# huakunyang/SummerTTS

Measured on AMD Instinct MI355X. Metric: audio samples/sec (acoustic model + vocoder, phoneme ids -> int16 PCM on host), single_speaker_fast-shaped synthetic blob, higher is better.
Workload: dtype f32 (decoder trunk convs AND the reverse flow's WaveNet convs (wn_flow.hip, one-utterance calls): fp32 operands as 2 fp16 terms = 22-23 of their 24 mantissa bits, 3 fp16 MFMA products per fp32 product, f32 accumulation -- measured error in `parity`, same tolerance as the exact-fp32 leg; batches addi

## Files before the change

### include/summertts_hip.h

```cpp
#ifndef SUMMERTTS_HIP_H_
#define SUMMERTTS_HIP_H_

#include <stdint.h>

#ifdef __cplusplus
extern "C" {
#endif

typedef struct sts_engine sts_engine;

enum {
    STS_OK = 0,
    STS_EINVAL = -1,
    STS_EMODEL = -2,
    STS_EDEVICE = -3,
    STS_ESTATE = -4
};

int sts_create(const float* blob, int64_t blob_bytes, int device, sts_engine** out);
void sts_destroy(sts_engine* e);

int sts_speaker_num(const sts_engine* e);

typedef struct sts_model_info {
// ... 126 lines not shown
#define STS_EQ_LOWPASS 5
typedef struct sts_eq_band { int32_t type; float freq_hz; float gain_db; float q; } sts_eq_band;
int sts_set_eq(sts_engine* e, int32_t n_bands, const sts_eq_band* bands);
int sts_get_eq(const sts_engine* e, int32_t* n_bands, sts_eq_band* bands, int32_t capacity);
int sts_eq_check(int32_t rate, int32_t n_bands, const sts_eq_band* bands);
int sts_eq_design(int32_t rate, int32_t n_bands, const sts_eq_band* bands, double* coeffs);
int sts_eq_apply(int device, const float* x, const int64_t* lengths, int32_t B, int32_t rate, int32_t n_bands,
                 const sts_eq_band* bands, float* y, int16_t* pcm);
int sts_set_eq_streaming(sts_engine* e, int enable);
int sts_get_eq_streaming(const sts_engine* e);
int sts_eq_apply_chunked(int device, const float* x, const int64_t* lengths, int32_t B, int32_t rate, int32_t n_bands,
                         const sts_eq_band* bands, const int64_t* bounds, int32_t n_steps, int32_t back, float* y, int16_t* pcm,
                         float* win_y, int64_t win_capacity, int64_t* win_off);
int sts_set_record_taps(sts_engine* e, int enable);
int sts_get_tap(sts_engine* e, const char* name, float** data, int32_t* channels, int64_t* length);
int sts_get_durations(sts_engine* e, int32_t* dur, int64_t capacity);
int sts_set_conv_mode(sts_engine* e, int mode);
int sts_set_conv_math(sts_engine* e, int mode);

enum { STS_DBG_ATTN_BLOCK_MIN_WGS = 1,
       STS_DBG_TAIL_FUSED = 14 ,
       STS_DBG_UPS_ROWPH = 15 ,
       STS_DBG_CHAIN_STREAMS = 13 ,
       STS_DBG_H2P = 11 ,
       STS_DBG_H2P_TILE = 12 ,
       STS_DBG_MEMO_CLEAR = 10 ,
       STS_DBG_PCM_DIRECT = 9 ,
       STS_DBG_DDS_TAIL = 8 ,
       STS_DBG_ATTN_REG = 7 ,
       STS_DBG_LAUNCH_AHEAD = 6 ,
       STS_DBG_FLOW_FUSED = 5  };
enum { STS_DBG_STREAM_RETRY_STEP = 16, STS_DBG_STREAM_DIRECT = 17 };
enum { STS_DBG_POISON = 18 };
int sts_debug_set(sts_engine* e, int key, int value);

typedef struct sts_profile {
    float ms_text_encoder, ms_duration, ms_flow, ms_decoder, ms_total_device;
    float ms_decoder_mfma;
    int32_t decoder_mfma_launches;
    double flops_text_encoder, flops_duration, flops_flow, flops_decoder;
    double flops_decoder_mfma;
    double bytes_decoder_min;
    int64_t frames, samples, phonemes;
    double flops_decoder_mfma_executed;
    double bytes_text_encoder, bytes_duration, bytes_flow;
    float ms_sync_wait_host;
    double flops_decoder_bf16_issued;
    int64_t conv_math_fallbacks;
    int32_t conv_math_pinned;
    int32_t launch_ahead;
    int64_t launch_ahead_misses;
    float us_host_setup;
    float us_host_enqueue;
    float us_host_tail;
    int64_t poison_bytes;
} sts_profile;
int sts_set_profiling(sts_engine* e, int enable);
#define STS_ABI_VERSION 16
int sts_abi_version(void);
int sts_build_flags(void);
int sts_get_profile(const sts_engine* e, sts_profile* p);
int sts_get_profile_ex(const sts_engine* e, void* p, int64_t size_bytes);

int sts_debug_conv1d(int device, const float* x, int32_t Cin, int32_t L, const float* w, const float* bias,
                     int32_t Cout, int32_t k, int32_t pad, int32_t dil, int32_t stride_transposed,
                     int32_t depthwise, float in_slope, int32_t in_act, int mode, float** y, int32_t* Lout);
// ... 97 lines not shown
```

### summertts_amd/csrc/capi.hip

```cpp
#include <stdlib.h>
#include <string.h>

#include <algorithm>
#include <new>
#include <string>
#include <utility>
#include <vector>

#include "engine.hpp"
#include "eq_stream.hpp"
#include "join_stream.hpp"
#include "loud_stream.hpp"

using namespace sts;

struct sts_engine { Engine eng; };

static thread_local std::string g_err;
static int set_err(int code, const std::string& s) { g_err = s; return code; }
#define STS_CAPI_NOT_WHILE_OPEN(e) \
    do { if ((e)->eng.stream_is_open()) return set_err(STS_ESTATE, "a stream is open on this engine (sts_stream_close first)"); } while (0)

extern "C" {

// ... 708 lines not shown
    if (noise_scale_w) *noise_scale_w = e->eng.noise.nsw;
    if (seed) *seed = e->eng.noise.seed;
    return STS_OK;
}
int sts_set_record_taps(sts_engine* e, int enable) { if (!e) return set_err(STS_EINVAL, "null engine"); STS_CAPI_NOT_WHILE_OPEN(e); e->eng.record_taps = enable != 0; return STS_OK; }
int sts_set_conv_math(sts_engine* e, int mode) {
    if (!e) return set_err(STS_EINVAL, "null engine");
    if (mode < 0 || mode > 3) return set_err(STS_EINVAL, "conv math: 0 = split-bf16 (default), 1 = exact fp32, 2 = split-bf16 wherever eligible, 3 = two-term fp16");
    STS_CAPI_NOT_WHILE_OPEN(e);
    e->eng.conv_math = mode;
    e->eng.h2_consecutive = 0; e->eng.h2_disabled = false;
    return STS_OK;
}
int sts_set_conv_mode(sts_engine* e, int mode) { if (!e) return set_err(STS_EINVAL, "null engine"); STS_CAPI_NOT_WHILE_OPEN(e); e->eng.conv_mode = mode; return STS_OK; }
int sts_debug_set(sts_engine* e, int key, int value) {
    if (!e) return set_err(STS_EINVAL, "null engine");
    if (key != STS_DBG_STREAM_RETRY_STEP && key != STS_DBG_POISON) STS_CAPI_NOT_WHILE_OPEN(e);
    switch (key) {
        case STS_DBG_ATTN_BLOCK_MIN_WGS: if (value < 1) return set_err(STS_EINVAL, "threshold must be >= 1"); e->eng.attn_block_min_wgs = value; return STS_OK;
        case STS_DBG_FLOW_FUSED: e->eng.flow_fused = value == 2 || value == 3 ? value : value != 0; return STS_OK;
        case STS_DBG_LAUNCH_AHEAD: if (value < 0 || value > 2) return set_err(STS_EINVAL, "launch_ahead must be 0, 1 or 2"); if ((value == 2) != (e->eng.launch_ahead == 2)) { e->eng.seen_tf_.clear(); e->eng.seen_order_.clear(); } e->eng.launch_ahead = value; return STS_OK;
        case STS_DBG_H2P: e->eng.h2p = value < 0 ? 0 : (value > 4 ? 4 : value); return STS_OK;
        case STS_DBG_H2P_TILE: e->eng.h2p_tile = value; return STS_OK;
        case STS_DBG_CHAIN_STREAMS: e->eng.chain_streams_dbg = value; return STS_OK;
        case STS_DBG_TAIL_FUSED: e->eng.tail_fused = value != 0; return STS_OK;
        case STS_DBG_UPS_ROWPH: e->eng.ups_rowph = value != 0; return STS_OK;
        case STS_DBG_MEMO_CLEAR: e->eng.seen_tf_.clear(); e->eng.seen_order_.clear(); return STS_OK;
        case STS_DBG_ATTN_REG: e->eng.attn_reg = value != 0; return STS_OK;
        case STS_DBG_DDS_TAIL: e->eng.dds_tail = value != 0; return STS_OK;
        case STS_DBG_PCM_DIRECT: e->eng.pcm_direct = value != 0; return STS_OK;
        case STS_DBG_STREAM_RETRY_STEP: e->eng.stream_retry_step = value < 0 ? -1 : value; return STS_OK;
        case STS_DBG_STREAM_DIRECT: e->eng.stream_direct = value != 0; return STS_OK;
        case STS_DBG_POISON: e->eng.poison = (unsigned)value; return STS_OK;
        default: return set_err(STS_EINVAL, "unknown debug key");
    }
}
int sts_set_host_pcm(sts_engine* e, int enable) { if (!e) return set_err(STS_EINVAL, "null engine"); e->eng.host_pcm = enable != 0; return STS_OK; }
int sts_set_profiling(sts_engine* e, int enable) { if (!e) return set_err(STS_EINVAL, "null engine"); e->eng.profiling = enable == 2 ? 2 : (enable != 0 ? 1 : 0); return STS_OK; }

int sts_abi_version(void) { return STS_ABI_VERSION; }

int sts_set_output_rate(sts_engine* e, int32_t rate) {
    if (!e) return set_err(STS_EINVAL, "null engine");
    const int rc = e->eng.set_output_rate(rate);
    return rc == STS_OK ? STS_OK : set_err(rc, e->eng.error());
}
int sts_get_output_rate(const sts_engine* e) {
    if (!e) return set_err(STS_EINVAL, "null engine");
    return e->eng.out_rate;
}
int sts_resample_table(int32_t in_rate, int32_t out_rate, int32_t* P, int32_t* Q, int32_t* taps, float* table, int64_t capacity_floats) {
    ResampleDesign d;
    if (!resample_design(in_rate, out_rate, &d)) return set_err(STS_EINVAL, "rates must be integers in [8000, 48000] with P = out / gcd(in, out) <= 1024");
    const int64_t need = (int64_t)d.P * 2 * d.K;
    if (table && capacity_floats < need) return set_err(STS_EINVAL, "table capacity below P * taps floats");
    if (P) *P = d.P;
    if (Q) *Q = d.Q;
    if (taps) *taps = 2 * d.K;
    if (table) resample_table(d, in_rate, out_rate, table);
    return STS_OK;
}
int sts_set_loudness(sts_engine* e, int mode, float target_lufs, float peak_dbfs) {
    if (!e) return set_err(STS_EINVAL, "null engine");
    const int rc = e->eng.set_loudness(mode, target_lufs, peak_dbfs);
    return rc == STS_OK ? STS_OK : set_err(rc, e->eng.error());
}
// ... 817 lines not shown
```

### summertts_amd/csrc/col_layer.hip

```cpp
#include "kernels.hpp"
#include "devmath.hpp"

#ifndef STS_EXP
#define STS_EXP 0
#endif

namespace sts {

typedef float f32x4 __attribute__((ext_vector_type(4)));

__device__ __forceinline__ int cl_seg_start(const SegView& s, int b) { return (s.off ? s.off[b] : s.ioff) * s.scale + b * s.extra; }
__device__ __forceinline__ int cl_seg_len(const SegView& s, int b) { return (s.off ? s.len[b] : s.ilen) * s.scale + s.extra; }

template <int NSUB, bool TAIL = false>
__global__ __launch_bounds__(64 * NSUB) void col_layer_kernel(ColLayerArgs a) {
    constexpr int C = 16 * NSUB, KQ = C / 4, CG = 4 * NSUB;
    constexpr int KH = KQ > 48 ? KQ / 2 : KQ;
    __shared__ float ys[C * 16];
    __shared__ float red[2][NSUB][16];
    const int b = blockIdx.y;
    const int len = cl_seg_len(a.seg, b);
    const int n0 = blockIdx.x * 16;
    if (n0 >= len) return;
    const size_t base = (size_t)cl_seg_start(a.seg, b);
// ... 128 lines not shown
    for (int r = 0; r < 4; r++) {
        float o = ((v[r] - mean) / den) * e_g[r] + e_b[r];
        if (a.post_gelu && !(STS_EXP & 1)) o = gelu_ref(o);
        if (a.res) o = e_res[r] + o;
        o4[r] = o;
        if (!TAIL) a.y[(size_t)(row0 + r) * a.y_ld + base + pos] = o;
    }
    if constexpr (TAIL) {
    __shared__ float tp[32 * 16], wb[32];
    __shared__ __attribute__((aligned(16))) float wl[C * 32];
#pragma unroll
    for (int r = 0; r < 4; r++) ys[(row0 + r) * 16 + col] = live ? o4[r] : 0.f;
    reinterpret_cast<f32x4*>(wl)[tid] = tw0; reinterpret_cast<f32x4*>(wl)[tid + 64 * NSUB] = tw1;
    if (tid < 32) wb[tid] = t_bias;
    __syncthreads();
    for (int j = tid >> 4; j < 32; j += 4 * NSUB) {
        float acc = 0.f;
#pragma unroll 8
        for (int c = 0; c < C; c++) acc += wl[c * 32 + j] * ys[c * 16 + col];
        acc += wb[j];
        tp[j * 16 + col] = j < 29 ? rq_spline_param(j, acc, a.tp_fs) : 0.f;
    }
    __syncthreads();
    if (tid < 16 && live) {
        float t[29];
#pragma unroll
        for (int j = 0; j < 29; j++) t[j] = tp[j * 16 + tid];
        a.tp_o0[base + pos] = rq_spline_inverse_t(t_in, t);
        a.tp_o1[base + pos] = t_keep;
    }
    }
}

template <int NSUB>
__global__ __launch_bounds__(64 * NSUB) void col_proj_kernel(ColProjArgs a) {
    constexpr int C = 16 * NSUB, KQ = C / 4, CG = 4 * NSUB;
    __shared__ float ys[C * 16];
    __shared__ float red[2][NSUB][16];
    const int b = blockIdx.y;
    const int len = cl_seg_len(a.seg, b);
    const int n0 = blockIdx.x * 16;
    if (n0 >= len) return;
    const size_t base = (size_t)cl_seg_start(a.seg, b);
    const int tid = threadIdx.x, lane = tid & 63, wave = tid >> 6;
    const int col = lane & 15, quad = lane >> 4;
    const int pos = n0 + col;
    const bool live = pos < len;
    const int cg = tid >> 4;

    float v[4], g[4], be[4];
    if (a.ids) {
        int id = live ? a.ids[base + pos] : 0;
        if (id < 0 || id >= a.vocab) id = 0;
#pragma unroll
        for (int i = 0; i < 4; i++) v[i] = live ? a.emb[(size_t)(cg + i * CG) * a.vocab + id] * a.emb_scale : 0.f;
    } else {
#pragma unroll
        for (int i = 0; i < 4; i++) {
            const int c = cg + i * CG;
            g[i] = a.gamma[c]; be[i] = a.beta[c];
            float x0 = live ? a.a[(size_t)c * a.a_ld + base + pos] : 0.f;
            float pb[8];
#pragma unroll
            for (int q = 0; q < 8; q++) pb[q] = (live && q < a.nb) ? a.bp[(size_t)q * a.b_stride + (size_t)c * a.b_ld + base + pos] : 0.f;
            float bs = pb[0];
#pragma unroll
            for (int q = 1; q < 8; q++) bs += pb[q];
            v[i] = x0 + bs;
        }
    }
    f32x4 afa[KQ / 4], afb[KQ / 4];
    auto load_strip = [&](int pass, f32x4 (&dst)[KQ / 4]) {
        const f32x4* wp = reinterpret_cast<const f32x4*>(a.wc) + ((size_t)pass * NSUB + wave) * (KQ / 4) * 64 + lane;
#pragma unroll
        for (int i = 0; i < KQ / 4; i++) dst[i] = wp[(size_t)i * 64];
    };
    load_strip(0, afa);

    if (!a.ids) {
        float s = 0.f, sq = 0.f;
#pragma unroll
        for (int i = 0; i < 4; i++) { s += v[i]; sq += v[i] * v[i]; }
        s += __shfl_xor(s, 16, 64); sq += __shfl_xor(sq, 16, 64);
        s += __shfl_xor(s, 32, 64); sq += __shfl_xor(sq, 32, 64);
        if (quad == 0) { red[0][wave][col] = s; red[1][wave][col] = sq; }
        __syncthreads();
        s = 0.f; sq = 0.f;
#pragma unroll
        for (int k = 0; k < NSUB; k++) { s += red[0][k][col]; sq += red[1][k][col]; }
        const float mean = s / (float)C;
        const float var = sq * (float)(1. / (float)C) - mean * mean;
        const float den = (float)sqrt((double)var + 1e-05);
#pragma unroll
        for (int i = 0; i < 4; i++) v[i] = ((v[i] - mean) / den) * g[i] + be[i];
    }
#pragma unroll
    for (int i = 0; i < 4; i++) {
        const int c = cg + i * CG;
        ys[c * 16 + col] = live ? v[i] : 0.f;
        if (live) a.x_out[(size_t)c * a.x_ld + base + pos] = v[i];
    }
    __syncthreads();

    float bq[KQ];
#pragma unroll
    for (int i = 0; i < KQ; i++) bq[i] = ys[(4 * i + quad) * 16 + col];
    const int rloc = wave * 16 + quad * 4;
    auto run_pass = [&](int pass, const f32x4 (&af)[KQ / 4]) {
        f32x4 acc0 = {0.f, 0.f, 0.f, 0.f}, acc1 = {0.f, 0.f, 0.f, 0.f};
#pragma unroll
        for (int i = 0; i < KQ; i += 2) {
            acc0 = __builtin_amdgcn_mfma_f32_16x16x4f32(af[i / 4][i % 4], bq[i], acc0, 0, 0, 0);
            acc1 = __builtin_amdgcn_mfma_f32_16x16x4f32(af[(i + 1) / 4][(i + 1) % 4], bq[i + 1], acc1, 0, 0, 0);
        }
        if (live) {
#pragma unroll
            for (int r = 0; r < 4; r++) {
                const int row = pass * C + rloc + r;
                if (row < a.Cout) a.y[(size_t)row * a.y_ld + base + pos] = (acc0[r] + acc1[r]) + (a.bias ? a.bias[row] : 0.f);
            }
        }
    };
    for (int pass = 0; pass < a.npass; pass += 2) {
        if (pass + 1 < a.npass) load_strip(pass + 1, afb);
        run_pass(pass, afa);
        if (pass + 1 < a.npass) {
            if (pass + 2 < a.npass) load_strip(pass + 2, afa);
            run_pass(pass + 1, afb);
        }
    }
}

bool col_proj_eligible(const ColProjArgs& a) {
    if (a.C != 32 && a.C != 64 && a.C != 192) return false;
    if (!a.wc || !a.y || !a.x_out || a.npass < 1 || a.npass > 4 || a.Cout > a.npass * a.C || a.Cout <= (a.npass - 1) * a.C) return false;
    if (a.ids) { if (!a.emb || a.vocab <= 0) return false; }
    else if (!a.a || !a.gamma || !a.beta || a.nb < 0 || a.nb > 8 || (a.nb > 0 && !a.bp)) return false;
    return a.max_len > 0 && a.B > 0;
}

void col_proj(const ColProjArgs& a, hipStream_t st) {
    const dim3 grid((a.max_len + 15) / 16, a.B);
    switch (a.C) {
        case 32: hipLaunchKernelGGL((col_proj_kernel<2>), grid, dim3(128), 0, st, a); break;
        case 64: hipLaunchKernelGGL((col_proj_kernel<4>), grid, dim3(256), 0, st, a); break;
        default: hipLaunchKernelGGL((col_proj_kernel<12>), grid, dim3(768), 0, st, a); break;
    }
}

void col_layer_pack(const float* w, int C, float* dst) { col_proj_pack(w, C, C, dst); }
void col_proj_pack(const float* w, int C, int Cout, float* dst) {
    const int nsub = C / 16, kq4 = C / 16, npass = (Cout + C - 1) / C;
    for (int pass = 0; pass < npass; pass++)
        for (int wave = 0; wave < nsub; wave++)
            for (int i4 = 0; i4 < kq4; i4++)
                for (int lane = 0; lane < 64; lane++)
                    for (int e = 0; e < 4; e++) {
                        const int co = pass * C + 16 * wave + (lane & 15), ci = 4 * (4 * i4 + e) + (lane >> 4);
                        dst[((((size_t)pass * nsub + wave) * kq4 + i4) * 64 + lane) * 4 + e] = co < Cout ? w[(size_t)co * C + ci] : 0.f;
                    }
}
bool col_layer_width_ok(int C) { return C == 32 || C == 64 || C == 192 || C == 256; }

bool col_layer_eligible(const ColLayerArgs& a) {
    if (!col_layer_width_ok(a.C)) return false;
    if (!a.wc || !a.g2 || !a.b2 || !a.x || !a.y) return false;
    if (a.dw_w && (!a.g1 || !a.b1 || a.dw_k < 1 || a.dw_k > 3)) return false;
    if (a.xs_w && (!a.dw_w || a.res != a.x)) return false;
    if (a.tp_w && (a.C == 256 || !a.tp_b || !a.tp_o0 || !a.tp_o1 || a.tp_o0 == a.tp_r0 || a.tp_o0 == a.tp_r1 || a.tp_o1 == a.tp_r1)) return false;
    if (a.y == a.x) return false;
    return a.max_len > 0 && a.B > 0;
}

void col_layer(const ColLayerArgs& a, hipStream_t st) {
// ... 19 lines not shown
```

### summertts_amd/csrc/engine.hip

```cpp
#include "run_ctx.hpp"
#include <time.h>
#include "knobs.hpp"
#include "../../include/tts_logger.h"

#include <algorithm>
#include <chrono>
#include <math.h>
#include <new>
#include <stdlib.h>
#include <string.h>
#include <thread>

namespace sts {

#define STS_NOT_WHILE_OPEN(what) \
    do { if (live_) return fail(STS_ESTATE, "a stream is open on this engine (sts_stream_close first): it refuses " what); } while (0)

Engine::~Engine() {
    if (live_) (void)stream_close();
    if (stream) (void)hipStreamSynchronize(stream);
    free_model(model);
    if (arenaT_.base) (void)hipFree(arenaT_.base);
    if (arenaF_.base) (void)hipFree(arenaF_.base);
    if (pinned_) (void)hipHostFree(pinned_);
// ... 561 lines not shown
    for (int b = 0; b < B; b++) { p_ns[b] = c.nz[b].ns; p_nsw[b] = c.nz[b].nsw; p_seed[b] = c.nz[b].seed; }
    int* p_ids = (int*)(p_seed + B);
    for (int b = 0; b < B; b++) memcpy(p_ids + offT[b], ids[b], sizeof(int) * n[b]);
    if (mix) memcpy(p_ids + Ttot, mix_words.data(), sizeof(int) * mix_ints);
    if (gain) memcpy(p_ids + Ttot + mix_ints, gain_words.data(), sizeof(int) * gain_ints);
    if (join) memcpy(p_ids + Ttot + mix_ints + gain_ints, join_sil.data(), sizeof(int) * join_ints);
    int* p_forced = p_ids + Ttot + mix_ints + gain_ints + join_ints;
    if (have_forced) memcpy(p_forced, forced_dur.data(), sizeof(int) * Ttot);
    if (plan) {
        memcpy(p_ids + Ttot + mix_ints + gain_ints + join_ints, plan_rate.data(), sizeof(float) * Ttot);
        memcpy(p_ids + 2 * Ttot + mix_ints + gain_ints + join_ints, plan_fixed.data(), sizeof(int) * Ttot);
        memcpy(p_ids + 3 * Ttot + mix_ints + gain_ints + join_ints, plan_target.data(), sizeof(int) * B);
    }
    HIPCK(hipMemcpyAsync(bt.meta_i, pm, (meta_ints + 5 * (size_t)B + (size_t)Ttot * (have_forced ? 2 : 1) + mix_ints + gain_ints + join_ints + plan_ints) * 4, hipMemcpyHostToDevice, stream));
    if (B > 1) HIPCK(hipEventRecord(ev_setup_, stream));

    static const bool no_inline_seg_knob = exp_flag("STS_NO_INLINE_SEG");
    const bool no_inline_seg = c.no_inline_seg = no_inline_seg_knob;
    const bool inl = c.inl = B == 1 && !no_inline_seg;
    c.ms = M.is_ms == 1;
    lvT.seg = inl ? SegView{nullptr, nullptr, 1, 0, 0, lenT[0]} : SegView{d_offT, d_lenT, 1, 0, 0, 0};
    Lvl& lvB = c.lvB; lvB = Lvl(); lvB.seg = no_inline_seg ? SegView{d_one, d_one + 1, 1, 0, 0, 0} : SegView{nullptr, nullptr, 1, 0, 0, B};
    lvB.nb = 1; lvB.max_len = B; lvB.total = B; lvB.ld = B;

    return STS_OK;
}

int Engine::run_text_encoder(RunCtx& c) {
    RUN_ALIASES(c)
    stage_begin(0);
    static const bool no_colp = exp_flag("STS_NO_COL_LAYER") || exp_flag("STS_NO_COL_PROJ");
    const long colp_blocks = (long)((Ttot + 15) / 16);
    const bool colp_grid = (long)((maxT + 15) / 16) * B <= 512;
    auto produce_x_and_conv = [&](int l, const DConv& c, float* y) {
        ColProjArgs pj;
        memset(&pj, 0, sizeof(pj));
        pj.x_out = bt.x; pj.x_ld = Ttot; pj.wc = c.wc; pj.bias = c.bias_rows; pj.Cout = c.Cout; pj.npass = (c.Cout + H - 1) / H;
        pj.y = y; pj.y_ld = Ttot; pj.C = H; pj.seg = lvT.seg; pj.B = B; pj.max_len = maxT;
        if (l == 0) { pj.ids = bt.ids; pj.emb = M.emb; pj.vocab = M.vocab; pj.emb_scale = sqrtf((float)M.hidden); }
        else { pj.a = bt.x1; pj.a_ld = Ttot; pj.bp = bt.y; pj.b_ld = Ttot; pj.nb = ffn2_slices; pj.b_stride = (long)H * Ttot;
               pj.gamma = M.ln2[l - 1].g; pj.beta = M.ln2[l - 1].b; }
        const bool ok = !no_colp && conv_mode != 1 && colp_grid && (pj.npass == 1 || colp_blocks >= 24) && c.k == 1 && c.Cin == H && M.emb_size == H && c.wc &&
                        (l == 0 || M.ln2[l - 1].C == H) && col_proj_eligible(pj);
        if (ok) {
            flops_[0] += 2.0 * c.macs_per_out * (double)Ttot;
            bytes_[0] += 4.0 * ((double)H * Ttot * (l == 0 ? 1.0 : 2.0 + ffn2_slices) + (double)c.Cout * Ttot + (double)H * c.Cout);
            col_proj(pj, stream);
            return;
        }
        if (l == 0) embed(bt.ids, M.emb, M.vocab, M.emb_size, sqrtf((float)M.hidden), bt.x, Ttot, (int)Ttot, stream);
        else ln(M.ln2[l - 1], bt.x1, bt.y, nullptr, bt.x, lvT, 0, 0, ffn2_slices, (long)H * Ttot);
        conv(c, bt.x, lvT, y, lvT, ConvOpt());
    };
    for (int l = 0; l < M.n_layers; l++) {
        const DMha& a = M.mha[l];
        produce_x_and_conv(l, a.qkv, bt.qkv);
        AttnArgs at;
        memset(&at, 0, sizeof(at));
        at.q = bt.qkv; at.k = bt.qkv + (size_t)H * Ttot; at.v = bt.qkv + (size_t)2 * H * Ttot; at.o = bt.att; at.ld = Ttot;
        at.relk = a.relk; at.relv = a.relv; at.kc = a.kc; at.px = a.px; at.win = a.win; at.nheads = 2;
        at.seg = lvT.seg; at.B = B; at.max_len = maxT; at.block_min_wgs = attn_block_min_wgs; at.attn_reg = attn_reg;
        attention(at, stream);
        flops_[0] += 2.0 * 2.0 * (double)a.ch * (double)maxT * (double)Ttot;
        bytes_[0] += 4.0 * 4.0 * (double)H * (double)Ttot;
        {
            static const bool no_col = exp_flag("STS_NO_COL_LAYER");
            ColLayerArgs g;
            memset(&g, 0, sizeof(g));
            g.x = bt.att; g.x_ld = Ttot; g.wc = a.o.wc; g.bias = a.o.bias;
            g.add = bt.x; g.add_ld = Ttot; g.g2 = M.ln1[l].g; g.b2 = M.ln1[l].b; g.y = bt.x1; g.y_ld = Ttot; g.C = H;
            g.seg = lvT.seg; g.B = B; g.max_len = maxT;
            if (!no_col && conv_mode != 1 && a.o.Cin == H && a.o.Cout == H && a.o.Cin_pad == H && M.ln1[l].C == H && col_layer_eligible(g)) {
                flops_[0] += 2.0 * a.o.macs_per_out * (double)Ttot;
                bytes_[0] += 4.0 * ((double)H * Ttot * 3.0 + (double)H * H);
                col_layer(g, stream);
            } else {
                conv(a.o, bt.att, lvT, bt.y, lvT, ConvOpt());
                ln(M.ln1[l], bt.x, bt.y, nullptr, bt.x1, lvT, 0, 0);
            }
// ... 1 lines not shown
        const DFfn& f = M.ffn[l];
        ConvOpt o1; o1.pad_l = f.ksize == 1 ? 0 : (f.ksize - 1) / 2;
        conv(f.c1, bt.x1, lvT, bt.ffh, lvT, o1);
        ConvOpt o2 = o1; o2.in_act = 1; o2.slope = 0.f;
        o2.kslices = ffn2_slices; o2.kslice_stride = (long)H * Ttot;
        conv(f.c2, bt.ffh, lvT, bt.y, lvT, o2);
    }
    produce_x_and_conv(M.n_layers, M.proj, bt.m);
    if (bt.logs) conv(M.proj_logs, bt.x, lvT, bt.logs, lvT, ConvOpt());
    tap("x_enc", bt.x, H, Ttot, Ttot);
    tap("m", bt.m, C, Ttot, Ttot);
    if (bt.logs) tap("logs", bt.logs, C, Ttot, Ttot);
    mark(1);
    return STS_OK;
}

int Engine::run_durations(RunCtx& c) {
    Model& M = model;
    const int B = c.B; const StreamSpec* const ss = c.ss; const long Ttot = c.Ttot;
    [[maybe_unused]] const int H = c.H, fdp = c.fdp;
    Lvl &lvT = c.lvT, &lvB = c.lvB; BufT& bt = c.bt;
    const size_t up_bytes = c.up_bytes; int* const pm = c.pm; int* const p_offF = c.p_offF; int* const p_lenF = c.p_lenF;
    int* const d_sid = c.d_sid; int* const d_offF = c.d_offF;
    const bool inl = c.inl, ms = c.ms; const int maxT = c.maxT; (void)maxT;

    stage_begin(1);
    if (ms && c.mix) speaker_blend(M.emb_g, M.spk_num, M.gin, d_sid, B, speaker_mix_tab(bt.mix, B, mix_K), bt.g, stream);
    else if (ms) gather_speaker(M.emb_g, M.spk_num, M.gin, d_sid, B, bt.g, stream);

    const float* r_final = nullptr;
    if (M.dur_type == 0) {
        ConvOpt op;
        if (ms) { conv(M.sdp_cond, bt.g, lvB, bt.cond_dp, lvB, ConvOpt()); op.ubias = bt.cond_dp; }
        conv(M.sdp_pre, bt.x, lvT, bt.dh, lvT, op);
        const float* dh = dds(M.sdp_dds, bt.dh, bt.dt1, bt.dt2, lvT);
        conv(M.sdp_proj, dh, lvT, bt.dc, lvT, ConvOpt());
        const float *r0 = nullptr, *r1 = nullptr;
        float *n0 = bt.dr[2], *n1 = bt.dr[3], *s0 = bt.dr[0], *s1 = bt.dr[1];
        if (c.any_nsw) { sdp_noise(lvT.seg, B, maxT, bt.nsw, bt.seed, bt.dr[0], bt.dr[1], stream); r0 = bt.dr[0]; r1 = bt.dr[1]; }
        else if (M.sdp_flows <= 1) { HIPCK(hipMemsetAsync(bt.dr[0], 0, (size_t)Ttot * 4, stream)); r0 = bt.dr[0]; }
        for (int i = M.sdp_flows - 1; i > 0; i--) {
            const DConvFlow& cf = M.cf[i];
            const SplineTail tl{&cf.proj, sqrtf((float)cf.filter), r0, r1, n0, n1};
            bool tail_done = false;
            const float* dhh = dds(cf.dds, bt.dhh, bt.dt1, bt.dt2, lvT, &cf.pre, r0, bt.dc, &tl, &tail_done);
            if (!tail_done) {
                conv(cf.proj, dhh, lvT, bt.dp29, lvT, ConvOpt());
                spline_step(bt.dp29, Ttot, sqrtf((float)cf.filter), r0, r1, n0, n1, Ttot, stream);
            }
            r0 = n0; r1 = n1;
            float* t;
            t = n0; n0 = s0; s0 = t;
            t = n1; n1 = s1; s1 = t;
        }
        r_final = r0;
    } else {
        const float* xin = bt.x;
        if (ms) {
            conv(M.fix_cond, bt.g, lvB, bt.cond_dp, lvB, ConvOpt());
            HIPCK(hipMemcpyAsync(bt.dh, bt.x, (size_t)H * Ttot * 4, hipMemcpyDeviceToDevice, stream));
            add_ubias(bt.dh, Ttot, bt.cond_dp, H, lvT.seg, B, maxT, stream);
            xin = bt.dh;
        }
        conv(M.fix_c1, xin, lvT, bt.dt1, lvT, ConvOpt());
        ln(M.fix_n1, bt.dt1, nullptr, nullptr, bt.dt1, lvT, 1, 0);
        conv(M.fix_c2, bt.dt1, lvT, bt.dt2, lvT, ConvOpt());
        ln(M.fix_n2, bt.dt2, nullptr, nullptr, bt.dt2, lvT, 1, 0);
// ... 1022 lines not shown
```

### summertts_amd/csrc/engine.hpp

```cpp
#pragma once
#include <hip/hip_runtime.h>

#include <deque>
#include <map>
#include <unordered_map>
#include <string>
#include <vector>

#include "../../include/summertts_hip.h"
#include "kernels.hpp"
#include "live_stream.hpp"
#include "model.hpp"

namespace sts {

struct Arena {
    char* base = nullptr; size_t cap = 0, used = 0; bool measuring = false;
    void* alloc(size_t bytes) {
        size_t a = (used + 255) & ~(size_t)255;
        used = a + bytes;
        if (measuring) return nullptr;
        return base + a;
    }
    template <typename T> T* get(size_t count) { return (T*)alloc(count * sizeof(T)); }
// ... 83 lines not shown
    int set_gain_plan(int B, const int32_t* n, const sts_gain_plan* plans);
    bool join_on = false; std::vector<int32_t> join_sil; long long join_total_sil = 0; int join_h = 0;
    std::vector<int64_t> last_join_start;
    int run_joined(int B, const int32_t* const* ids, const int32_t* n, const int32_t* sid, const float* ls, const sts_join* join, const StreamSpec* ss = nullptr);
    int join_offsets(int64_t* start, int64_t capacity);
    std::vector<int32_t> last_n;
    int phoneme_offsets(int64_t* start, int64_t capacity);
    bool record_taps = false; int profiling = 0;
    int conv_mode = 0;
    int conv_math = 3;
    long h2_fallbacks = 0;
    int h2_consecutive = 0; bool h2_disabled = false;
    double products() const { return conv_math == 3 ? 3.0 : 6.0; }
    int pcm_direct = 1;
    int dds_tail = 1;
    int attn_reg = 1;
    int attn_block_min_wgs = 96;
    int launch_ahead = 1;
    long ahead_misses = 0;
    static constexpr size_t kMemoEntries = 1024;
    std::unordered_map<unsigned long long, long> seen_tf_; std::deque<unsigned long long> seen_order_;
    bool polite_wait = false;
    struct WaitEst { double us = 0.0; long phonemes = 0; };
    WaitEst wait_est_[2][24];
    void nap_before_wait(int which, long phonemes);
    void note_wait(int which, long phonemes, double waited_us, bool was_ready_at_wake);
    int final_sync(long phonemes);
    int ups_rowph = 1;
    int tail_fused = 1;
    int chain_streams_dbg = -1;
    int h2p = 1;
    int h2p_tile = -1;
    int flow_fused = 1;
    int n_cus = 0;
    int stream_retry_step = -1;
    int stream_direct = 0;
    unsigned poison = 0;
    int64_t poison_bytes_ = 0;
    hipStream_t stream = nullptr;

private:
    int fail(int code, const std::string& msg) { err_ = msg; return code; }
    bool ensure(Arena& a, size_t bytes);
    bool ensure_pinned(size_t bytes);
    void poison_arena(const Arena& a);
    void poison_host16(void* p, size_t samples);
    void poison_host32(void* p, size_t words);
    ConvArgs conv_args(const DConv& c, const float* x, const Lvl& lin, float* y, const Lvl& lout, const ConvOpt& o, double* flops);
    void conv(const DConv& c, const float* x, const Lvl& lin, float* y, const Lvl& lout, const ConvOpt& o);
    void ln(const DLn& l, const float* a, const float* b, const float* res, float* y, const Lvl& lv, int pre_relu, int post_gelu, int nb = 1, long b_stride = 0);
    int pick_kslices(const DConv& c, const Lvl& lout) const;
    struct SplineTail { const DConv* proj; float filter_sqrt; const float* r0; const float* r1; float* o0; float* o1; };
    float* dds(const DDds& d, float* h, float* t1, float* t2, const Lvl& lv, const DConv* pre = nullptr, const float* pre_in = nullptr,
               const float* pre_res = nullptr, const SplineTail* tail = nullptr, bool* tail_done = nullptr);
    int run_any_math(int B, const int32_t* const* ids, const int32_t* n, const int32_t* sid, const float* ls, const StreamSpec* ss);
    struct RunCtx;
    struct ResStage;
    int run_setup(RunCtx& c);
    int run_text_encoder(RunCtx& c);
    int run_durations(RunCtx& c);
    int run_frame_workspace(RunCtx& c);
    int run_flow(RunCtx& c);
    int run_decode(RunCtx& c, int nw, long Wtot, int maxW, int zoff0, int wlen0);
    int decode_end(RunCtx& c, const float* wave, const WinGeom& win, long Wtot, int maxW);
    int wait_frame_counts(RunCtx& c);
    int plan_output(RunCtx& c);
// ... 56 lines not shown
```

### summertts_amd/csrc/kernels.hpp

```cpp
#pragma once
#include <hip/hip_runtime.h>
#include <stdint.h>

#include <vector>

#include "../../include/summertts_hip.h"

namespace sts {

struct SegView {
    const int* off;
    const int* len;
    int scale;
    int extra;
    int ioff, ilen;
};

enum Epilogue : int {
    EPI_STORE = 0,
    EPI_RESADD = 1,
    EPI_SUB = 3,
    EPI_GATE = 4,
    EPI_RESSKIP = 5,
    EPI_TANH_PCM = 6,
// ... 47 lines not shown
};

struct ColLayerArgs {
    const float* x; long x_ld;
    const float* xs_w; const float* xs_b; const float* xr;
    const float* dw_w; const float* dw_b; int dw_k, dw_dil, dw_pad, dw_ld;
    const float* g1; const float* b1;
    const float* wc; const float* bias;
    const float* add; long add_ld;
    const float* g2; const float* b2; int post_gelu;
    const float* res; long res_ld;
    float* y; long y_ld;
    int C;
    SegView seg; int B, max_len;
    const float* tp_w; const float* tp_b;
    float tp_fs;
    const float* tp_r0; const float* tp_r1;
    float* tp_o0; float* tp_o1;
};
bool col_layer_eligible(const ColLayerArgs& a);
bool col_layer_width_ok(int C);
void col_layer_pack(const float* w, int C, float* dst);
void col_layer(const ColLayerArgs& a, hipStream_t st);

struct ColProjArgs {
    const int* ids; const float* emb; int vocab; float emb_scale;
    const float* a; long a_ld; const float* bp; long b_ld; int nb; long b_stride;
    const float* gamma; const float* beta;
    float* x_out; long x_ld;
    const float* wc; const float* bias; int Cout, npass;
    float* y; long y_ld;
    int C;
    SegView seg; int B, max_len;
};
bool col_proj_eligible(const ColProjArgs& a);
void col_proj(const ColProjArgs& a, hipStream_t st);
void col_proj_pack(const float* w, int C, int Cout, float* dst);

struct AttnArgs {
    const float* q; const float* k; const float* v; float* o; long ld;
    const float* relk; const float* relv;
    int kc, px, win, nheads;
    SegView seg; int B, max_len;
    int block_min_wgs;
    int attn_reg;
};


struct FlowLayerArgs {
    SegView seg; int B, max_len; long tot;
    int H, half, G, Cg, k, halo;
    int layer;
    const float* x0; long x0_ld; const float* pend; int pend_n; long pend_stride; float* x0_out; long x0_out_ld;
    const void* w_pre; const float* b_pre; float s_pre;
    const float* h_in; const float* part_in; int part_n; long part_stride;
    float* h_out;
    float* part_out;
    float* macc; long macc_stride; int macc_init;
    const void* w_gate; const float* b_gate; float s_gate;
    const float* ubias; int ubias_ld;
    const void* w_c; float s_c; int rows_c, rows_res;
    const float* b_res; const float* b_m;
    unsigned* ovf;
};
struct FlowFinishArgs {
    SegView seg; int B, max_len; int half;
// ... 262 lines not shown
```

### summertts_amd/csrc/model.hip

```cpp
#include "model.hpp"
#include "kernels.hpp"

#include <hip/hip_runtime.h>
#include <math.h>
#include <string.h>

namespace sts {

namespace {

struct Reader {
    const float* p; int64_t n; int64_t o = 0; bool ok = true;
    int geti() { if (o >= n) { ok = false; return 0; } return (int)p[o++]; }
    const float* take(int64_t cnt) {
        if (cnt < 0 || o + cnt > n) { ok = false; return p; }
        const float* r = p + o; o += cnt; return r;
    }
};

HConv parse_conv(Reader& r) {
    HConv c;
    c.out_ch = r.geti(); c.in_ch = r.geti(); c.k = r.geti(); c.pad = r.geti(); c.dil = r.geti(); c.has_bias = r.geti();
    if (c.out_ch <= 0 || c.in_ch <= 0 || c.k <= 0 || c.out_ch > (1 << 20) || c.in_ch > (1 << 20) || c.k > 4096) { r.ok = false; return c; }
    c.w = r.take((int64_t)c.in_ch * c.k * c.out_ch);
// ... 534 lines not shown
            if (h.in_ch != w.H || h.out_ch != 2 * w.H || h.k != wk) FAIL("WN in_layer shape");
            h.pad = (wk * dil - dil) / 2; h.dil = dil;
            PackOpts o; o.gate = true; o.gate_H = w.H;
            if (!pack_conv(st, h, o, w.in[l]) || !pack_bf3(st, w.in[l])) FAIL("WN in_layer pack");
        }
        for (int l = 0; l < w.n; l++) {
            HConv h = parse_conv(r);
            if (!r.ok || h.k != 1 || h.in_ch != w.H || (h.out_ch != 2 * w.H && h.out_ch != w.H)) FAIL("WN res_skip");
            if ((l < w.n - 1) != (h.out_ch == 2 * w.H)) FAIL("WN res_skip shape");
            if (!pack_conv(st, h, PackOpts(), w.rs[l]) || !pack_bf3(st, w.rs[l])) FAIL("WN res_skip pack");
            w.rs[l].H = w.H;
        }
        w.has_cond = m.is_ms == 1;
        if (w.has_cond) {
            HConv h = parse_conv(r);
            if (!r.ok || h.out_ch != 2 * w.H * w.n) FAIL("WN cond_layer");
            PackOpts o; o.gate_blocks = true; o.gate_H = w.H;
            if (!pack_conv(st, h, o, w.cond)) FAIL("WN cond pack");
        }
        HConv post = parse_conv(r);
        if (!r.ok || post.k != 1 || post.out_ch != m.inter / 2 || post.in_ch != w.H || pre.out_ch != w.H) FAIL("coupling post");
        { PackOpts o; o.reverse_out = c.flipped; if (!pack_conv(st, post, o, c.post) || !pack_bf3(st, c.post)) FAIL("coupling post pack"); }
        if (!pack_flow_fused(st, c)) FAIL("coupling fused-layer pack");
    }

    if (m.dur_type == 0) {
        m.sdp_flows = r.geti();
        if (!r.ok || m.sdp_flows < 2 || m.sdp_flows > 64) FAIL("sdp flows");
        { const float* e = r.take(4); if (!r.ok) FAIL("sdp affine"); m.ea_m = e[0]; m.ea_logs = e[2]; }
        m.cf.resize(m.sdp_flows);
        for (int i = 0; i < m.sdp_flows; i++) if (!parse_pack_convflow(r, st, m.cf[i])) FAIL("sdp ConvFlow");
        parse_conv(r); parse_conv(r); skip_dds(r); r.take(4);
        for (int i = 0; i < 4; i++) skip_convflow(r);
        { HConv h = parse_conv(r); if (!r.ok || h.k != 1 || !pack_conv(st, h, PackOpts(), m.sdp_pre)) FAIL("sdp pre"); }
        { HConv h = parse_conv(r); if (!r.ok || h.k != 1 || !pack_conv(st, h, PackOpts(), m.sdp_proj)) FAIL("sdp proj"); }
        if (!parse_pack_dds(r, st, m.sdp_dds)) FAIL("sdp dds");
        if (m.is_ms == 1) { HConv h = parse_conv(r); if (!r.ok || !pack_conv(st, h, PackOpts(), m.sdp_cond)) FAIL("sdp cond"); }
    } else {
        { HConv h = parse_conv(r); if (!r.ok || !pack_conv(st, h, PackOpts(), m.fix_c1)) FAIL("fix conv_1"); }
        { HLn h = parse_ln(r); if (!r.ok || !pack_ln(st, h, m.fix_n1)) FAIL("fix norm_1"); }
        { HConv h = parse_conv(r); if (!r.ok || !pack_conv(st, h, PackOpts(), m.fix_c2)) FAIL("fix conv_2"); }
        { HLn h = parse_ln(r); if (!r.ok || !pack_ln(st, h, m.fix_n2)) FAIL("fix norm_2"); }
        { HConv h = parse_conv(r); if (!r.ok || h.out_ch != 1 || !pack_conv(st, h, PackOpts(), m.fix_proj)) FAIL("fix proj"); }
        if (m.is_ms == 1) { HConv h = parse_conv(r); if (!r.ok || !pack_conv(st, h, PackOpts(), m.fix_cond)) FAIL("fix cond"); }
    }
    if (m.is_ms == 1) {
        m.spk_num = r.geti(); m.gin = r.geti();
        if (!r.ok || m.spk_num <= 0 || m.gin <= 0) FAIL("speaker table header");
        const float* e = r.take((int64_t)m.spk_num * m.gin);
        if (!r.ok || !copy_raw(st, e, (size_t)m.spk_num * m.gin, &m.emb_g)) FAIL("speaker table");
    }
    if (!r.ok) FAIL("blob truncated");
    m.consumed = r.o;
    { const float* slack; if (!st.alloc(1024, &slack)) FAIL("weight store overflow"); }
    m.dev_floats = st.used;
    if (!st.commit()) FAIL("mapping device memory behind the weight store failed");
    m.dev_mapped = st.mapped; m.dev_handle = st.vmm ? (void*)st.handle : nullptr;
    if (hipMemcpy(st.dev, st.host.data(), st.used * sizeof(float), hipMemcpyHostToDevice) != hipSuccess) FAIL("weight upload failed");
    return true;
}

void free_model(Model& m) {
    if (m.dev_weights) {
        if (m.dev_vmm) {
            if (m.dev_mapped) { (void)hipMemUnmap(m.dev_weights, m.dev_mapped); (void)hipMemRelease((hipMemGenericAllocationHandle_t)m.dev_handle); }
            (void)hipMemAddressFree(m.dev_weights, m.dev_reserved);
        } else (void)hipFree(m.dev_weights);
// ... 6 lines not shown
```

### summertts_amd/csrc/run_ctx.hpp

```cpp
#pragma once
#include "engine.hpp"
#include "eq_stream.hpp"
#include "loud_stream.hpp"
#include "out_chain.hpp"
#include "join_stream.hpp"
#include "stream_step.hpp"

namespace sts {

#define HIPCK(call)                                                                           \
    do {                                                                                      \
        hipError_t e__ = (call);                                                              \
        if (e__ != hipSuccess) return fail(STS_EDEVICE, std::string(#call) + ": " + hipGetErrorString(e__)); \
    } while (0)

struct BufT {
    int *meta_i; float* ls; float *ns, *nsw; uint64_t* seed; int* ids; int* forced;
    float *x, *qkv, *att, *y, *x1, *ffh, *m, *logs;
    float *dh, *dt1, *dt2, *dc, *dhh, *dp29, *dr[4], *dlogw;
    int *dur, *cum, *frames;
    float *g, *cond_dp, *cond_dec, *cond_wn;
    float* plan_rate; int *plan_fixed, *plan_target; long long* plan_rem; float* dur_w;
    int* mix;
    int *gain_q, *gain_h;
    int* join_sil;
};
struct BufF {
    float *z, *h, *acts, *out, *x0, *regA, *regB, *tailA, *tailB, *tailC, *wave, *fliptmp;
    float *ff_h[2], *ff_part[2], *ff_macc[2], *ff_alt;
    int16_t* pcm;
    int16_t* pcm_nat; float* wave_out;
    int16_t* pcm_rs; char* lws;
    char* limws; float* wave_lim;
    float* wave_gain;
    float* wave_join;
    char* stab; int16_t* spack; float *gwin, *cond_win;
    float* wave_eq; char* eqws;
    char* eqst; double* eqsE;
    char* ldst; double* ldsE; char* ldres;
};
struct Engine::RunCtx {
    int B = 0; const int32_t* const* ids = nullptr; const int32_t* n = nullptr; const int32_t* sid = nullptr; const float* ls = nullptr;
    const StreamSpec* ss = nullptr;
    std::vector<int> offT, lenT; long Ttot = 0; int maxT = 0;
    int H = 0, C = 0, FF = 0, fdp = 0, wnH = 0, wnL = 0, ffn2_slices = 1;
    Lvl lvT, lvB, lv1;
    BufT bt; BufF bf;
    size_t meta_ints = 0, up_bytes = 0;
    int *pm = nullptr, *p_offT = nullptr, *p_lenT = nullptr, *p_sid = nullptr, *p_offF = nullptr, *p_lenF = nullptr, *p_one = nullptr;
    int *d_offT = nullptr, *d_lenT = nullptr, *d_sid = nullptr, *d_offF = nullptr, *d_lenF = nullptr, *d_one = nullptr, *d_win = nullptr;
    bool inl = false, no_inline_seg = false, ms = false;
    long Ftot = 0; int maxF = 0, hop = 0;
    long Fld = 0; int maxFld = 0; bool ahead = false, ahead_b = false, mapped = false, forced = false;
    bool plan = false;
    bool gain = false;
    bool join = false;
    long long FJ = 0;
    bool mix = false;
    std::vector<Engine::Noise> nz; bool any_ns = false, any_nsw = false;
    std::vector<unsigned long long> req_keys; std::vector<long> predF;
    int halo = 0; long Wcap = 0; int upS = 1; long Lsb = 0; int sbC = 0;
    long long Ocap = 0;
    bool bstream = false;
    bool use_ff = false; int ffG = 0, ffNT = 32;
    OutChain oc{}; LimiterDesign limd; int rsP = 1, rsQ = 1, eqS = 0;
    const float* stage_out(int s) const {
        const float* const o[OS_COUNT] = {bf.wave, bf.wave_gain, bf.wave_join, bf.wave_out, nullptr, bf.wave_eq, nullptr, bf.wave_lim};
        return s < 0 ? nullptr : o[s];
    }
    JsPlan js;
    LiveStream* live = nullptr; std::vector<int> live_slots;
};
#define RUN_ALIASES(c)                                                                                                              \
    [[maybe_unused]] Model& M = model;                                                                                              \
    [[maybe_unused]] const int B = (c).B; [[maybe_unused]] const StreamSpec* const ss = (c).ss;                                     \
    [[maybe_unused]] const long Ttot = (c).Ttot; [[maybe_unused]] const int maxT = (c).maxT;                                        \
    [[maybe_unused]] const int H = (c).H, C = (c).C, FF = (c).FF, fdp = (c).fdp, wnH = (c).wnH, wnL = (c).wnL, ffn2_slices = (c).ffn2_slices; \
    [[maybe_unused]] Lvl &lvT = (c).lvT, &lvB = (c).lvB, &lv1 = (c).lv1;                                                            \
    [[maybe_unused]] BufT& bt = (c).bt; [[maybe_unused]] BufF& bf = (c).bf;                                                         \
    [[maybe_unused]] const size_t up_bytes = (c).up_bytes;                                                                          \
    [[maybe_unused]] int* const pm = (c).pm; [[maybe_unused]] int* const p_offF = (c).p_offF; [[maybe_unused]] int* const p_lenF = (c).p_lenF; \
    [[maybe_unused]] int* const d_sid = (c).d_sid; [[maybe_unused]] int* const d_offF = (c).d_offF; [[maybe_unused]] int* const d_lenF = (c).d_lenF; \
    [[maybe_unused]] int* const d_win = (c).d_win;                                                                                  \
    [[maybe_unused]] const bool inl = (c).inl, no_inline_seg = (c).no_inline_seg, ms = (c).ms;                                      \
// ... 8 lines not shown
```

### summertts_amd/engine.py

```python
from __future__ import annotations

import ctypes as C
import os
import subprocess
from typing import Dict, List, Optional, Sequence

import numpy as np

_HERE = os.path.dirname(os.path.abspath(__file__))
LIB_PATH = os.environ.get("SUMMERTTS_HIP_LIB") or os.path.join(_HERE, "lib", "libsummertts_hip.so")
CSRC = os.path.join(_HERE, "csrc")


def build_library(verbose: bool = False) -> str:
    subprocess.run(["make", "-C", CSRC, "-j8"], check=True, stdout=None if verbose else subprocess.DEVNULL)
    return LIB_PATH


class ModelInfo(C.Structure):
    _fields_ = [("is_multi_speaker", C.c_int32), ("lang_type", C.c_int32), ("dur_pred_type", C.c_int32),
                ("dec_type", C.c_int32), ("vocab", C.c_int32), ("hidden", C.c_int32), ("inter_channels", C.c_int32),
                ("speaker_num", C.c_int32), ("gin_channels", C.c_int32), ("samples_per_frame", C.c_int32),
                ("sample_rate", C.c_int32), ("blob_floats_consumed", C.c_int64)]

# ... 1008 lines not shown
    def get_eq_streaming(self) -> bool:
        return bool(self.lib.sts_get_eq_streaming(self.h))

    def get_eq(self):
        n = C.c_int32()
        arr = (EqBand * EQ_MAX_BANDS)()
        _check(self.lib, self.lib.sts_get_eq(self.h, C.byref(n), arr, EQ_MAX_BANDS))
        return [(int(arr[i].type), float(arr[i].freq_hz), float(arr[i].gain_db), float(arr[i].q)) for i in range(n.value)]

    def limiter_mode(self):
        m, g, c, l = C.c_int(), C.c_float(), C.c_float(), C.c_float()
        _check(self.lib, self.lib.sts_get_limiter_mode(self.h, C.byref(m), C.byref(g), C.byref(c), C.byref(l)))
        return m.value, g.value, c.value, l.value

    def limiter(self) -> np.ndarray:
        n = self.lib.sts_get_limiter(self.h, None, 0)
        if n < 0:
            _check(self.lib, n)
        out = np.zeros(n, LIMITER_DTYPE)
        if n:
            rc = self.lib.sts_get_limiter(self.h, out.ctypes.data, n)
            if rc < 0:
                _check(self.lib, rc)
        return out

    def set_conv_math(self, mode):
        m = {"bf16x3": 0, "f32": 1, "bf16x3_all": 2, "f16x2": 3}.get(mode, mode)
        _check(self.lib, self.lib.sts_set_conv_math(self.h, int(m)))

    def set_conv_mode(self, mode: int):
        _check(self.lib, self.lib.sts_set_conv_mode(self.h, mode))

    def debug_set(self, key: str, value: int):
        _check(self.lib, self.lib.sts_debug_set(self.h, {"attn_block_min_wgs": 1, "flow_fused": 5, "launch_ahead": 6, "attn_reg": 7, "dds_tail": 8, "pcm_direct": 9, "memo_clear": 10, "h2p": 11, "h2p_tile": 12, "chain_streams": 13, "tail_fused": 14, "ups_rowph": 15, "stream_retry_step": 16, "stream_direct": 17, "poison": 18}[key], int(value)))

    def set_profiling(self, on):
        _check(self.lib, self.lib.sts_set_profiling(self.h, 2 if on == 2 else (1 if on else 0)))

    def profile(self) -> dict:
        p = Profile()
        _check(self.lib, self.lib.sts_get_profile_ex(self.h, C.byref(p), C.sizeof(p)))
        return p.as_dict()

    def tap(self, name: str) -> np.ndarray:
        ptr = C.POINTER(C.c_float)()
        ch, ln = C.c_int32(), C.c_int64()
        _check(self.lib, self.lib.sts_get_tap(self.h, name.encode(), C.byref(ptr), C.byref(ch), C.byref(ln)))
        a = np.ctypeslib.as_array(ptr, shape=(ch.value, ln.value)).copy()
        self.lib.sts_free(ptr)
        return a

    def durations(self, total_phonemes: int) -> np.ndarray:
        d = np.zeros(total_phonemes, np.int32)
        _check(self.lib, self.lib.sts_get_durations(self.h, d.ctypes.data, d.size))
        return d

    def close(self):
        if getattr(self, "h", None) is not None and self.h:
            self.lib.sts_destroy(self.h)
            self.h = None

    def __del__(self):
        try:
            self.close()
        except Exception:
            pass

# ... 412 lines not shown
```

Before: 66.60 million.

## Split col_proj passes across grid z and fold sdp_pre conv into encoder's last projection

```diff
diff --git a/include/summertts_hip.h b/include/summertts_hip.h
--- a/include/summertts_hip.h
+++ b/include/summertts_hip.h
@@ -182,6 +182,7 @@
        STS_DBG_FLOW_FUSED = 5  };
 enum { STS_DBG_STREAM_RETRY_STEP = 16, STS_DBG_STREAM_DIRECT = 17 };
 enum { STS_DBG_POISON = 18 };
+enum { STS_DBG_COL_PROJ = 19, STS_DBG_SDP_PRE_RIDE = 20 };
 int sts_debug_set(sts_engine* e, int key, int value);
 
 typedef struct sts_profile {
diff --git a/summertts_amd/csrc/capi.hip b/summertts_amd/csrc/capi.hip
--- a/summertts_amd/csrc/capi.hip
+++ b/summertts_amd/csrc/capi.hip
@@ -764,6 +764,8 @@
         case STS_DBG_STREAM_RETRY_STEP: e->eng.stream_retry_step = value < 0 ? -1 : value; return STS_OK;
         case STS_DBG_STREAM_DIRECT: e->eng.stream_direct = value != 0; return STS_OK;
         case STS_DBG_POISON: e->eng.poison = (unsigned)value; return STS_OK;
+        case STS_DBG_COL_PROJ: if (value < 0 || value > 3) return set_err(STS_EINVAL, "col_proj must be 0, 1, 2 or 3"); e->eng.col_proj_mode = value; return STS_OK;
+        case STS_DBG_SDP_PRE_RIDE: e->eng.sdp_pre_ride = value != 0; return STS_OK;
         default: return set_err(STS_EINVAL, "unknown debug key");
     }
 }
diff --git a/summertts_amd/csrc/col_layer.hip b/summertts_amd/csrc/col_layer.hip
--- a/summertts_amd/csrc/col_layer.hip
+++ b/summertts_amd/csrc/col_layer.hip
@@ -184,7 +184,7 @@
     }
 }
 
-template <int NSUB>
+template <int NSUB, bool SPLIT = false>
 __global__ __launch_bounds__(64 * NSUB) void col_proj_kernel(ColProjArgs a) {
     constexpr int C = 16 * NSUB, KQ = C / 4, CG = 4 * NSUB;
     __shared__ float ys[C * 16];
@@ -199,6 +199,11 @@
     const int pos = n0 + col;
     const bool live = pos < len;
     const int cg = tid >> 4;
+    const float* wsel = a.wc; const float* bsel = a.bias; float* ysel = a.y; long yld = a.y_ld; int cout = a.Cout, pass0 = 0;
+    if constexpr (SPLIT) {
+        pass0 = blockIdx.z;
+        if (pass0 >= a.npass) { wsel = a.wc2; bsel = a.bias2; ysel = a.y2; yld = a.y2_ld; cout = a.Cout2; pass0 = 0; }
+    }
 
     float v[4], g[4], be[4];
     if (a.ids) {
@@ -221,13 +226,13 @@
             v[i] = x0 + bs;
         }
     }
-    f32x4 afa[KQ / 4], afb[KQ / 4];
+    f32x4 afa[KQ / 4];
     auto load_strip = [&](int pass, f32x4 (&dst)[KQ / 4]) {
-        const f32x4* wp = reinterpret_cast<const f32x4*>(a.wc) + ((size_t)pass * NSUB + wave) * (KQ / 4) * 64 + lane;
+        const f32x4* wp = reinterpret_cast<const f32x4*>(wsel) + ((size_t)pass * NSUB + wave) * (KQ / 4) * 64 + lane;
 #pragma unroll
         for (int i = 0; i < KQ / 4; i++) dst[i] = wp[(size_t)i * 64];
     };
-    load_strip(0, afa);
+    load_strip(pass0, afa);
 
     if (!a.ids) {
         float s = 0.f, sq = 0.f;
@@ -250,7 +255,7 @@
     for (int i = 0; i < 4; i++) {
         const int c = cg + i * CG;
         ys[c * 16 + col] = live ? v[i] : 0.f;
-        if (live) a.x_out[(size_t)c * a.x_ld + base + pos] = v[i];
+        if (live && (!SPLIT || blockIdx.z == 0)) a.x_out[(size_t)c * a.x_ld + base + pos] = v[i];
     }
     __syncthreads();
 
@@ -269,16 +274,21 @@
 #pragma unroll
             for (int r = 0; r < 4; r++) {
                 const int row = pass * C + rloc + r;
-                if (row < a.Cout) a.y[(size_t)row * a.y_ld + base + pos] = (acc0[r] + acc1[r]) + (a.bias ? a.bias[row] : 0.f);
+                if (row < cout) ysel[(size_t)row * yld + base + pos] = (acc0[r] + acc1[r]) + (bsel ? bsel[row] : 0.f);
             }
         }
     };
-    for (int pass = 0; pass < a.npass; pass += 2) {
-        if (pass + 1 < a.npass) load_strip(pass + 1, afb);
-        run_pass(pass, afa);
-        if (pass + 1 < a.npass) {
-            if (pass + 2 < a.npass) load_strip(pass + 2, afa);
-            run_pass(pass + 1, afb);
+    if constexpr (SPLIT) {
+        run_pass(pass0, afa);
+    } else {
+        f32x4 afb[KQ / 4];
+        for (int pass = 0; pass < a.npass; pass += 2) {
+            if (pass + 1 < a.npass) load_strip(pass + 1, afb);
+            run_pass(pass, afa);
+            if (pass + 1 < a.npass) {
+                if (pass + 2 < a.npass) load_strip(pass + 2, afa);
+                run_pass(pass + 1, afb);
+            }
         }
     }
 }
@@ -288,10 +298,20 @@
     if (!a.wc || !a.y || !a.x_out || a.npass < 1 || a.npass > 4 || a.Cout > a.npass * a.C || a.Cout <= (a.npass - 1) * a.C) return false;
     if (a.ids) { if (!a.emb || a.vocab <= 0) return false; }
     else if (!a.a || !a.gamma || !a.beta || a.nb < 0 || a.nb > 8 || (a.nb > 0 && !a.bp)) return false;
+    if (a.wc2 && (!a.split || !a.y2 || a.Cout2 < 1 || a.Cout2 > a.C)) return false;
     return a.max_len > 0 && a.B > 0;
 }
 
 void col_proj(const ColProjArgs& a, hipStream_t st) {
+    if (a.split) {
+        const dim3 grid((a.max_len + 15) / 16, a.B, a.npass + (a.wc2 ? 1 : 0));
+        switch (a.C) {
+            case 32: hipLaunchKernelGGL((col_proj_kernel<2, true>), grid, dim3(128), 0, st, a); break;
+            case 64: hipLaunchKernelGGL((col_proj_kernel<4, true>), grid, dim3(256), 0, st, a); break;
+            default: hipLaunchKernelGGL((col_proj_kernel<12, true>), grid, dim3(768), 0, st, a); break;
+        }
+        return;
+    }
     const dim3 grid((a.max_len + 15) / 16, a.B);
     switch (a.C) {
         case 32: hipLaunchKernelGGL((col_proj_kernel<2>), grid, dim3(128), 0, st, a); break;
diff --git a/summertts_amd/csrc/engine.hip b/summertts_amd/csrc/engine.hip
--- a/summertts_amd/csrc/engine.hip
+++ b/summertts_amd/csrc/engine.hip
@@ -617,6 +617,8 @@
     static const bool no_colp = exp_flag("STS_NO_COL_LAYER") || exp_flag("STS_NO_COL_PROJ");
     const long colp_blocks = (long)((Ttot + 15) / 16);
     const bool colp_grid = (long)((maxT + 15) / 16) * B <= 512;
+    bool& dh_in_enc = c.dh_in_enc;
+    dh_in_enc = false;
     auto produce_x_and_conv = [&](int l, const DConv& c, float* y) {
         ColProjArgs pj;
         memset(&pj, 0, sizeof(pj));
@@ -625,11 +627,23 @@
         if (l == 0) { pj.ids = bt.ids; pj.emb = M.emb; pj.vocab = M.vocab; pj.emb_scale = sqrtf((float)M.hidden); }
         else { pj.a = bt.x1; pj.a_ld = Ttot; pj.bp = bt.y; pj.b_ld = Ttot; pj.nb = ffn2_slices; pj.b_stride = (long)H * Ttot;
                pj.gamma = M.ln2[l - 1].g; pj.beta = M.ln2[l - 1].b; }
-        const bool ok = !no_colp && conv_mode != 1 && colp_grid && (pj.npass == 1 || colp_blocks >= 24) && c.k == 1 && c.Cin == H && M.emb_size == H && c.wc &&
+        const bool one_launch = pj.npass == 1 || col_proj_mode != 0;
+        pj.split = pj.npass > 1 && (col_proj_mode == 3 || (col_proj_mode == 1 && colp_blocks < 24));
+        const DConv& sp = M.sdp_pre;
+        const bool ride = l == M.n_layers && sdp_pre_ride && M.dur_type == 0 && !ms && sp.k == 1 && sp.Cin == H && sp.Cout == H && sp.wc;
+        if (ride) { pj.split = 1; pj.wc2 = sp.wc; pj.bias2 = sp.bias_rows; pj.y2 = bt.dh; pj.y2_ld = Ttot; pj.Cout2 = sp.Cout; }
+        const bool ok = !no_colp && conv_mode != 1 && colp_grid && one_launch && c.k == 1 && c.Cin == H && M.emb_size == H && c.wc &&
                         (l == 0 || M.ln2[l - 1].C == H) && col_proj_eligible(pj);
         if (ok) {
+            const int zs = pj.split ? pj.npass + (ride ? 1 : 0) : 1;
             flops_[0] += 2.0 * c.macs_per_out * (double)Ttot;
-            bytes_[0] += 4.0 * ((double)H * Ttot * (l == 0 ? 1.0 : 2.0 + ffn2_slices) + (double)c.Cout * Ttot + (double)H * c.Cout);
+            bytes_[0] += 4.0 * ((double)H * Ttot * (1.0 + zs * (l == 0 ? 0.0 : 1.0 + ffn2_slices)) + (double)c.Cout * Ttot + (double)H * c.Cout);
+            if (ride) {
+                flops_[1] += 2.0 * sp.macs_per_out * (double)Ttot;
+                bytes_[1] += 4.0 * ((double)sp.Cin * Ttot + (double)sp.Cout * Ttot);
+                bytes_w_[1] += 4.0 * (double)sp.Cin * sp.Cout;
+                dh_in_enc = true;
+            }
             col_proj(pj, stream);
             return;
         }
@@ -697,7 +711,7 @@
     if (M.dur_type == 0) {
         ConvOpt op;
         if (ms) { conv(M.sdp_cond, bt.g, lvB, bt.cond_dp, lvB, ConvOpt()); op.ubias = bt.cond_dp; }
-        conv(M.sdp_pre, bt.x, lvT, bt.dh, lvT, op);
+        if (!c.dh_in_enc) conv(M.sdp_pre, bt.x, lvT, bt.dh, lvT, op);
         const float* dh = dds(M.sdp_dds, bt.dh, bt.dt1, bt.dt2, lvT);
         conv(M.sdp_proj, dh, lvT, bt.dc, lvT, ConvOpt());
         const float *r0 = nullptr, *r1 = nullptr;
diff --git a/summertts_amd/csrc/engine.hpp b/summertts_amd/csrc/engine.hpp
--- a/summertts_amd/csrc/engine.hpp
+++ b/summertts_amd/csrc/engine.hpp
@@ -139,6 +139,8 @@
     int h2p = 1;
     int h2p_tile = -1;
     int flow_fused = 1;
+    int col_proj_mode = 1;
+    int sdp_pre_ride = 1;
     int n_cus = 0;
     int stream_retry_step = -1;
     int stream_direct = 0;
diff --git a/summertts_amd/csrc/kernels.hpp b/summertts_amd/csrc/kernels.hpp
--- a/summertts_amd/csrc/kernels.hpp
+++ b/summertts_amd/csrc/kernels.hpp
@@ -103,6 +103,8 @@
     float* y; long y_ld;
     int C;
     SegView seg; int B, max_len;
+    int split;
+    const float* wc2; const float* bias2; float* y2; long y2_ld; int Cout2;
 };
 bool col_proj_eligible(const ColProjArgs& a);
 void col_proj(const ColProjArgs& a, hipStream_t st);
diff --git a/summertts_amd/csrc/model.hip b/summertts_amd/csrc/model.hip
--- a/summertts_amd/csrc/model.hip
+++ b/summertts_amd/csrc/model.hip
@@ -590,7 +590,7 @@
         for (int i = 0; i < m.sdp_flows; i++) if (!parse_pack_convflow(r, st, m.cf[i])) FAIL("sdp ConvFlow");
         parse_conv(r); parse_conv(r); skip_dds(r); r.take(4);
         for (int i = 0; i < 4; i++) skip_convflow(r);
-        { HConv h = parse_conv(r); if (!r.ok || h.k != 1 || !pack_conv(st, h, PackOpts(), m.sdp_pre)) FAIL("sdp pre"); }
+        { HConv h = parse_conv(r); if (!r.ok || h.k != 1 || !pack_conv(st, h, PackOpts(), m.sdp_pre) || !pack_col(st, h, m.sdp_pre)) FAIL("sdp pre"); }
         { HConv h = parse_conv(r); if (!r.ok || h.k != 1 || !pack_conv(st, h, PackOpts(), m.sdp_proj)) FAIL("sdp proj"); }
         if (!parse_pack_dds(r, st, m.sdp_dds)) FAIL("sdp dds");
         if (m.is_ms == 1) { HConv h = parse_conv(r); if (!r.ok || !pack_conv(st, h, PackOpts(), m.sdp_cond)) FAIL("sdp cond"); }
diff --git a/summertts_amd/csrc/run_ctx.hpp b/summertts_amd/csrc/run_ctx.hpp
--- a/summertts_amd/csrc/run_ctx.hpp
+++ b/summertts_amd/csrc/run_ctx.hpp
@@ -50,6 +50,7 @@
     int *pm = nullptr, *p_offT = nullptr, *p_lenT = nullptr, *p_sid = nullptr, *p_offF = nullptr, *p_lenF = nullptr, *p_one = nullptr;
     int *d_offT = nullptr, *d_lenT = nullptr, *d_sid = nullptr, *d_offF = nullptr, *d_lenF = nullptr, *d_one = nullptr, *d_win = nullptr;
     bool inl = false, no_inline_seg = false, ms = false;
+    bool dh_in_enc = false;
     long Ftot = 0; int maxF = 0, hop = 0;
     long Fld = 0; int maxFld = 0; bool ahead = false, ahead_b = false, mapped = false, forced = false;
     bool plan = false;
diff --git a/summertts_amd/engine.py b/summertts_amd/engine.py
--- a/summertts_amd/engine.py
+++ b/summertts_amd/engine.py
@@ -1064,7 +1064,7 @@
         _check(self.lib, self.lib.sts_set_conv_mode(self.h, mode))
 
     def debug_set(self, key: str, value: int):
-        _check(self.lib, self.lib.sts_debug_set(self.h, {"attn_block_min_wgs": 1, "flow_fused": 5, "launch_ahead": 6, "attn_reg": 7, "dds_tail": 8, "pcm_direct": 9, "memo_clear": 10, "h2p": 11, "h2p_tile": 12, "chain_streams": 13, "tail_fused": 14, "ups_rowph": 15, "stream_retry_step": 16, "stream_direct": 17, "poison": 18}[key], int(value)))
+        _check(self.lib, self.lib.sts_debug_set(self.h, {"attn_block_min_wgs": 1, "flow_fused": 5, "launch_ahead": 6, "attn_reg": 7, "dds_tail": 8, "pcm_direct": 9, "memo_clear": 10, "h2p": 11, "h2p_tile": 12, "chain_streams": 13, "tail_fused": 14, "ups_rowph": 15, "stream_retry_step": 16, "stream_direct": 17, "poison": 18, "col_proj": 19, "sdp_pre_ride": 20}[key], int(value)))
 
     def set_profiling(self, on):
         _check(self.lib, self.lib.sts_set_profiling(self.h, 2 if on == 2 else (1 if on else 0)))
```

Result: faster. 67.74 million, median of 6 (+1.7%).
